# eflynn8/pharmacophore-diffusion

Measured on AMD Instinct MI355X. Metric: denoising steps/sec (batch x T) at 256-atom pocket, 6 centers, higher is better.
Workload: dtype f32; 1 GPU; BASELINE config 2: 256-atom pocket, 6 centers, T=500 schedule, batch=32 per GPU, dev.yml network; batch_per_gpu=32, n_prot=256, n_pharm=6, T=500, parallelism=graphs sharded over 1 GPU(s), no data-path collective

## Files before the change

pharmacophore-diffusion_amd/csrc/pf_device.h:

```cpp
#pragma once
#include <stdint.h>

#define PF_S 128
#define PF_V 16
#define PF_R 16
#define PF_MAXF 64
#define PF_MAXK 16
#define PF_MAX_GVPS 8

enum { ET_FF = 0, ET_PF = 1, ET_FP = 2, ET_PP = 3 };

#if defined(__HIP_DEVICE_COMPILE__)
#define PF_AS1 __attribute__((address_space(1)))
#else
#define PF_AS1
#endif
typedef const float PF_AS1* pf_gcf;

struct GvpW {
    pf_gcf a_wh;
    pf_gcf a_wu;
    pf_gcf a_main;
    pf_gcf a_main_c;
    pf_gcf a_gate_c;
// ... 105 lines not shown
    const float4* xn;
    const float* h;
    const float* v;
    float* msg_s;
    float* msg_v;
    const GvpW* w;
    const float* pre;
    int n_gvps;
    float rbf_mu[PF_R];
    float rbf_inv_sigma;
    float* sv_z; float* sv_g; float* sv_v; size_t sv_stride;
    int bf16;
    pf_gcf rg[4];
    const int* reg; int nreg, regB, ngroups4, ngroups8;
    pf_gcf rgs[4]; int rgs_stride;
    const float* zs;
    const float* ptab;
    int ptab_gstride;
    const int* ptype;
    const int* eorig;
    const int* l0_gid;
    const float* l0c;
    int ngroups_sel;
    const int* need; int need_stamp;
    int pa_abs;
    pf_gcf n16[4]; int n16_stride[4];
    int uni_base[3], uni_s01, uni_s2g, uni_pa_groups;
    int ptab16_off[4];
    const float* pcen; int pcen_nf;
    const float* x0_static;
    const int* pa_skip;
    int* cnt_snap;
    int* pa_gstamp; int pa_serial;
};

#define L0H_WR 0
#define L0H_WSH 2048
#define L0H_B 4224
#define L0H_WH0 4352
#define L0H_WU 4384
#define L0H_BG 4672
#define L0H_WHT 4736
#define L0H_WHT_PF 21120
#define L0H_B_PF 37504
#define L0H_SIZE (37504 + 128)
#define L0C_WHT_FF 0
#define L0C_B_FF 16384
#define L0C_WHT_FP 16512
#define L0C_B_FP 32896
#define L0C_SIZE (32896 + 128)
#define L0_NTAB 4
struct L0HoistParams {
    const float* src;
    float* l0c;
    const int* esrc; const int* edst; const float4* xn; int Epp;
    float rbf_mu0, rbf_mu_step, rbf_inv_sigma;
    float* zs;
    const float* enc_w; const float* enc_b; const float* enc_lw; const float* enc_lb;
    int rec_nf, nt;
    const float* t_dev;
    float t_host[64];
    float* ptab;
    const float* prot_h0; int Np; int* ptype; int* flag;
};

struct NodeW {
// ... 280 lines not shown
```

pharmacophore-diffusion_amd/csrc/pf_host.cpp:

```cpp
#include <hip/hip_runtime.h>

#include <algorithm>
#include <cmath>
#include <cstdio>
#include <cstdlib>
#include <cstring>
#include <ctime>
#include <map>
#include <string>
#include <unordered_map>
#include <climits>
#include <vector>

#include "../../include/pfdyn.h"
#include "pf_device.h"
#include "pf_bind.h"
#include "pf_pack.h"
#include "pf_train.h"
#include "pf_score.h"

using namespace pfpack;

#define L0_PTAB_SLOTS 2048

// ... 75 lines not shown
void pfk_drop_masks(const TrainCommon* c, uint32_t stream, int n_elems, float* out, hipStream_t s);
void pfk_pp_radius(const float4* xn, const int* prot_ptr, int B, float r2, int maxn, int* deg, const int* row_off,
                   int* src, int* dst, int pass, hipStream_t s);
void pfk_wide_encode(const WideEncParams* p, hipStream_t s);
void pfk_wide_pack(const float* flat, const WidePackJob* jobs, int n_jobs, float* out, hipStream_t s);
void pfk_wide_edge(const WideEdgeParams* p, int train, hipStream_t s);
void pfk_wide_node(const WideNodeParams* p, int train, hipStream_t s);
void pfk_wt_chain(const WtChainParams* p, int edge, int wgrad, hipStream_t s);
void pfk_wt_norm(const WtNormParams* p, int wgrad, hipStream_t s);
void pfk_wt_head_out(const WtHeadOutParams* p, int wgrad, hipStream_t s);
void pfk_wt_encode(const WtEncParams* p, int wgrad, hipStream_t s);
void pfk_wt_center_sum(const WtCenterSumParams* p, hipStream_t s);
void pfk_wt_reduce(const float* gpart, int gstride, float* grad, int nparams, hipStream_t s);
}

namespace {

static std::string g_create_error;

static void linspace_f32(float start, float end, int steps, float* out) {
    const float step = (end - start) / (float)(steps - 1);
    const int half = steps / 2;
    for (int i = 0; i < steps; ++i) out[i] = i < half ? start + step * (float)i : end - step * (float)(steps - i - 1);
}

}

struct LaunchPolicy {
    static constexpr int kCUs = 256, kSIMDs = 4 * kCUs;
    int n16_mask = 7;
    int tail_graphs_max = 256;
    int xcd_split = 1;
    int edge_rec = 1;
    int node_static = 1;
    int node_xcds = 2;
    int fused_uni = 1;
    int xchg_sleep = 1, hsb_avoid = 0;
    int hs_build = 1;
    int tail_form = 4;
    long n16_fuse_rows_max = 20000;
    long n16_rows_max = 24000;
    int rg_rows_max = 1 << 30;
    int rg2_rows_min = 12000;
    int rg2_rows_min_node = 12000;
    int rg2p_rows_min = 11000;
    int rg2_rows_min_hoist = 30000;
    int l0_rga = 0, l0_rgp = 0;
    int rg_split_max = 128;
    int rg_split_max_node = 256;
    int rg_split_max_head = 512;
    int coop_edge_max = 256, coop_node_max = 1024;
    int coop2_edge_max = 12000, coop2_dense_max = 1024;
    int rg_mode(int ntiles) const {
        const long rows = (long)ntiles * 32;
        if (rows > rg_rows_max) return 0;
        return rows >= rg2_rows_min ? 2 : 1;
    }
    void from_env() {
        auto geti = [](const char* v, int& x) { if (const char* e = getenv(v)) x = atoi(e); };
        geti("PFDYN_COOP_EDGE_MAX", coop_edge_max); geti("PFDYN_COOP_NODE_MAX", coop_node_max);
        if (const char* e = getenv("PFDYN_COOP2_EDGE_MAX")) coop2_edge_max = coop2_dense_max = atoi(e);
        if (const char* e = getenv("PFDYN_RG_SPLIT_MAX")) rg_split_max = rg_split_max_node = rg_split_max_head = atoi(e);
        geti("PFDYN_RG_SPLIT_MAX_NODE", rg_split_max_node); geti("PFDYN_RG_SPLIT_MAX_HEAD", rg_split_max_head);
        geti("PFDYN_RG_ROWS_MAX", rg_rows_max);
        if (const char* e = getenv("PFDYN_RG2_ROWS_MIN")) rg2_rows_min = rg2_rows_min_hoist = rg2p_rows_min = rg2_rows_min_node = atoi(e);
        geti("PFDYN_RG2P_ROWS_MIN", rg2p_rows_min); geti("PFDYN_RG2_ROWS_MIN_NODE", rg2_rows_min_node); geti("PFDYN_RG2_ROWS_MIN_HOIST", rg2_rows_min_hoist);
        geti("PFDYN_L0_RGP", l0_rgp); geti("PFDYN_L0_RGA", l0_rga);
        for (const char* v : {"PFDYN_RG2_ROWS_MIN", "PFDYN_RG2P_ROWS_MIN", "PFDYN_RG2_ROWS_MIN_HOIST", "PFDYN_RG_SPLIT_MAX", "PFDYN_L0_RGA",
                              "PFDYN_L0_RGP", "PFDYN_RG_ROWS_MAX"})
            if (getenv(v)) n16_mask = 0;
        geti("PFDYN_N16", n16_mask);
        geti("PFDYN_TAIL_GRAPHS_MAX", tail_graphs_max);
        geti("PFDYN_XCD_SPLIT", xcd_split);
        geti("PFDYN_EDGE_REC", edge_rec);
        geti("PFDYN_NODE_XCDS", node_xcds); geti("PFDYN_NODE_STATIC", node_static); geti("PFDYN_HS_BUILD", hs_build); geti("PFDYN_FUSED_UNI", fused_uni); geti("PFDYN_XCHG_SLEEP", xchg_sleep); geti("PFDYN_HSB_AVOID", hsb_avoid);
        if (const char* e = getenv("PFDYN_TAIL_FORM")) tail_form = (e[0] == 'n' || atoi(e) == 16) ? 16 : 4;
        if (const char* e = getenv("PFDYN_N16_ROWS_MAX")) n16_rows_max = n16_fuse_rows_max = atol(e);
        if (const char* e = getenv("PFDYN_N16_FUSE_ROWS_MAX")) n16_fuse_rows_max = atol(e);
    }
};

enum RunKind { RUN_NONE = 0, RUN_PLAIN, RUN_PINNED, RUN_GUIDED };

struct pf_handle {
    LaunchPolicy pol;
    pf_config cfg{};
    bool spec = true, wide = false;
    WideGvp* d_wgvp = nullptr;
    std::string err;
    std::map<std::string, RawTensor> raw;
    bool committed = false;

    float* d_w = nullptr;
    PackLayout pk;
    GvpW* d_gvp = nullptr;
    std::vector<GvpW> h_gvp;
    int msg_base(int layer, int et) const { return ((layer * 4 + et) * cfg.n_message_gvps); }
    int upd_base(int layer, int nt) const { return n_msg_tot + (layer * 2 + nt) * cfg.n_update_gvps; }
    int head_base() const { return n_msg_tot + n_upd_tot; }
    int n_msg_tot = 0, n_upd_tot = 0;
    bool use_pre = true;

    bool have_batch = false;
    int B = 0, Np = 0, Nf = 0, N = 0;
    int64_t Epp = 0, Ecap = 0;
    std::vector<int> h_prot_ptr, h_pharm_ptr;
    std::vector<int> h_reg;
// ... 37 lines not shown
    bool share_ok = false;
    int share_check = 1;
    int* d_reg_share = nullptr;
    int* d_pa_static = nullptr;
    int* d_rep_base = nullptr;
    int* d_need = nullptr;
    int need_stamp = 0, edges_stamp = 0;
    long share_rows = 0;
    std::vector<int> h_share_start, h_share_cnt;
    bool share_disable = false;
    bool train_rg_node = true;
    bool train_rg_edge = true;
    bool train_rg_head = true;
    float *t_hsv_z = nullptr, *t_hsv_g = nullptr, *t_hsv_v = nullptr;
    bool t_head_saved = false;
    unsigned int* d_xchg = nullptr;
    int* d_xstat = nullptr;
    int* xstat_host = nullptr;
    int xstat_ack = 0;
    int xchg_fault = 0, xchg_poll_max = 0;
    bool cen_hoist = true;
    float *d_cen_h = nullptr, *d_cen_p = nullptr, *d_snap[2] = {nullptr, nullptr};
    unsigned int* d_xchg2 = nullptr;
    int snap_cur = -1;
    std::vector<float> t_plan; size_t plan_pos = 0;
    bool cen_valid = false; float cen_t = 0.f; uint64_t cen_wver = 0;
    bool last_cen = false;
    bool pa_spec = true;
    bool spec_valid = false; float spec_t = 0.f; uint64_t spec_wver = 0;
    int step_id = 2;
    int *d_pa_stamp = nullptr, *d_pa_same = nullptr;
    bool e0_saved = false; EdgeParams e0{}; EncodeParams ep0{}; int e0_groups = 0;
    int last_spec = 0;
    int* d_pa_cnt = nullptr;
    int pa_spec_split = 0;
    bool pa_check = false;
    int pa_serial = 0, spec_serial = 0;
    int* d_pa_gstamp = nullptr;
    unsigned long long* d_pa_chk = nullptr;
    bool no_fixed_shapes = false;
    ScaleArgs pend_scale{}; bool has_pend_scale = false;
    bool vjp_full_kernels = false;
    bool no_fix_fuse = false;
    bool train_bf16 = false;
    bool train_node_save = true;
    std::vector<float*> t_nsv_z, t_nsv_g, t_nsv_v;
    std::vector<char> t_node_saved;
    std::vector<int> t_grp;
    RunKind run = RUN_NONE;
    void* d_pin = nullptr; size_t pin_capacity = 0;
    int* d_pin_flags = nullptr; float *d_pin_x = nullptr, *d_pin_h = nullptr;
    float pin_feat_norm = 1.f;
    void* d_seed = nullptr; size_t seed_capacity = 0;
    float *d_seed_x = nullptr, *d_seed_h = nullptr;
    float seed_alpha = 1.f, seed_sigma = 0.f, seed_feat_norm = 1.f;
    bool seed_armed = false;
    void* d_restr = nullptr; size_t restr_capacity = 0;
    void* restr_stage = nullptr; size_t restr_stage_capacity = 0; hipEvent_t restr_ev = nullptr;
    int n_restr = 0;
    float guide_scale = 0.f, guide_clip = 0.f;
    void* d_guide = nullptr; size_t guide_capacity = 0;
    float *d_g0 = nullptr, *d_gjx = nullptr, *d_ggrad = nullptr, *d_gshift = nullptr, *d_gzero = nullptr, *d_genergy = nullptr, *d_gD = nullptr;
    bool guide_have = false;
    float* guide_traj_energy = nullptr;
    int max_np = 0, max_nf = 0;
    bool edges_built = false;
// ... 401 lines not shown
        size_t total = 0;
        auto frag = [](int n_out, int K) { return (size_t)((n_out + 15) / 16) * ((K + 3) / 4) * 64; };
        for_each_gvp(c, [&](const GvpSpec& g) {
            const int H = std::max(g.vi, g.vo);
            const int* o = &h->po.gvp[6 * tab.size()];
            WideGvp w{};
            w.wh = h->d_flat + o[0]; w.wu = h->d_flat + o[1]; w.bm = h->d_flat + o[3]; w.bg = h->d_flat + o[5];
            w.vi = g.vi; w.vo = g.vo; w.si = g.si; w.so = g.so;
            jobs.push_back({o[2], g.so, g.si + H, (int)total});
            total += frag(g.so, g.si + H);
            jobs.push_back({o[4], g.vo, g.so, (int)total});
            total += frag(g.vo, g.so);
            tab.push_back(w);
        });
        if (total >= (size_t)1 << 31) PF_FAIL(h, PF_ERR_ARG, "pf_train_set_family: the model is too large for the width-generic packing");
        if (h->d_wpk) { (void)hipFree(h->d_wpk); h->d_wpk = nullptr; }
        PF_HIP(h, hipMalloc((void**)&h->d_wpk, std::max<size_t>(total, 1) * sizeof(float)));
        PF_HIP(h, upload(&h->d_wpk_jobs, jobs));
        h->n_wpk_jobs = (int)jobs.size();
        for (size_t i = 0; i < tab.size(); ++i) { tab[i].wm = h->d_wpk + jobs[2 * i].dst; tab[i].wg = h->d_wpk + jobs[2 * i + 1].dst; }
        PF_HIP(h, upload(&h->d_wgvp, tab));
        h->wpk_version = ~0ull;
    }
    if (h->wpk_version != h->w_version) {
        pfk_wide_pack(h->d_flat, h->d_wpk_jobs, h->n_wpk_jobs, h->d_wpk, s);
        h->wpk_version = h->w_version;
    }
    return PF_OK;
}

static int run_dynamics_wide(pf_handle* h, float* eps_h, float* eps_x, hipStream_t s, const float* t_scalar, bool train = false) {
    const pf_config& c = h->cfg;
    h->tail_done = false; h->last_tail = 0; h->last_hoist = 0;
    h->cen_valid = false; h->last_cen = false; h->spec_valid = false; h->last_spec = 0; h->e0_saved = false;
    if (!train && h->share_ok && h->share_check == 0) (void)share_now(h);
    if (!train && h->share_check == 2)
        PF_FAIL(h, PF_ERR_ARG, "pf_set_pocket_groups: the claim made for this batch is false -- a graph differs from its representative in "
                               "coordinates or features (compared on the device); bind the batch again without the claim");
    const int rc = ensure_wide_pack(h, s);
    if (rc) return rc;
    const int S = c.n_hidden_scalars, V = c.vector_size;
    WideEncParams ep{};
    ep.Np = h->Np; ep.Nf = h->Nf; ep.S = S; ep.rec_nf = c.rec_nf; ep.pharm_nf = c.pharm_nf;
    ep.prot_h0 = h->d_prot_h0; ep.pharm_h = h->d_pharm_h;
    ep.t = t_scalar ? nullptr : h->d_t; ep.t_scalar = t_scalar ? *t_scalar : 0.f; ep.gid = h->d_gid;
    for (int nt = 0; nt < 2; ++nt) {
        ep.w[nt] = h->d_w + h->pk.enc_w[nt]; ep.b[nt] = h->d_w + h->pk.enc_b[nt];
        ep.ln_w[nt] = h->d_w + h->pk.enc_lw[nt]; ep.ln_b[nt] = h->d_w + h->pk.enc_lb[nt];
    }
    float* const* st_h = train ? h->wt.st_h : h->d_h;
    float* const* st_v = train ? h->wt.st_v : h->d_v;
    ep.h_out = st_h[0];
    { ProfScope ps(h, pf_handle::K_ENCODE, s); pfk_wide_encode(&ep, s); }
    if (!h->edges_built) {
        const BuildParams bp = build_params(h, false);
        { ProfScope ps(h, pf_handle::K_BUILD, s); pfk_build_edges(&bp, s); }
        build_done(h, false);
    }
    h->last_family.assign(c.n_convs, 64);
    if (train) pfk_copy(reinterpret_cast<const float*>(h->d_xn), h->wt.xkeep, (size_t)h->N * 4, s);
    int cur = 0;
    for (int l = 0; l < c.n_convs; ++l) {
        const bool last = l == c.n_convs - 1;
        const LayerTiles lt = layer_tiles(h, l);
        WideEdgeParams e{};
        e.tiles = lt.etiles; e.ntiles = lt.n_etiles;
        e.dyn_cnt = h->d_dyn_cnt; e.esrc = h->d_esrc; e.edst = h->d_edst; e.xn = h->d_xn;
// ... 105 lines not shown
    } else {
        L0HoistParams lp = l0_params(h);
        lp.nt = h->B; lp.t_dev = h->d_t; lp.ptab = h->d_ptab_pg;
        pfk_l0_hoist(&lp, 1, s);
        dc.l0_ptab = h->d_ptab_pg; dc.l0_gstride = L0_NTAB * c.rec_nf * PF_S;
    }
}
static void edge_n16_form(DynCall& dc, int l) {
    pf_handle* h = dc.h; EdgeParams& e = dc.e; const pf_config& c = h->cfg; const bool shared = dc.shared;
    for (int et = 0; et < 4; ++et) {
        e.n16[et] = h->d_w + (l > 0 ? h->pk.n16_msg[(size_t)l * 4 + et] : h->pk.n16_l0[et]);
        e.n16_stride[et] = (int)(l > 0 ? h->pk.n16_msg_stride : h->pk.n16_l0_stride[et]);
        e.ptab16_off[et] = et == ET_PP ? c.rec_nf * PF_S : (et == ET_PF ? 2 * c.rec_nf * PF_S : -1);
    }
    if (l == 0) { e.zs = nullptr; dc.rgp = 4; h->last_hoist = 16; }
    if (l == 0 && dc.step != nullptr && h->run != RUN_NONE && !h->coords_custom) {
        e.x0_static = h->d_prot_x0;
        if (dc.spec_have && pa_ahead_ok(h, e, shared)) { e.pa_skip = h->d_pa_same; h->last_spec = 1; }
    }
    if (l == 0 && dc.cen_have && h->pk.n16_l0h[ET_FF] != 0) {
        for (int et : {(int)ET_FF, (int)ET_FP}) { e.n16[et] = h->d_w + h->pk.n16_l0h[et]; e.n16_stride[et] = (int)h->pk.n16_l0h_stride[et]; }
        e.pcen = h->d_cen_p; e.pcen_nf = h->Nf; h->last_cen = true;
    }
    e.ngroups_sel = region_groups(h, shared, 0, e.nreg, 16);
    int stride[3], cap[3], grp[3] = {0, 0, 0};
    bool uni = l == 0 && h->pol.fused_uni && !shared && e.reg == h->d_reg && e.nreg == 4 * h->B && h->B <= 64 && !e.pa_abs && !e.need &&
               uniform_regions(h, 3, stride, cap);
    for (int et = 0; et < 3 && uni; ++et) { grp[et] = (cap[et] + 15) / 16; uni = grp[et] > 0 && grp[et] < 8; }
    if (uni) {
        for (int et = 0; et < 3; ++et) e.uni_base[et] = h->h_reg[(size_t)et * h->B];
        e.uni_s01 = stride[0] | (stride[1] << 16);
        e.uni_s2g = stride[2] | (grp[0] << 16) | (grp[1] << 19) | (grp[2] << 22) | ((h->B - 1) << 25);
        e.uni_pa_groups = region_groups(h, shared, 3 * h->B, 4 * h->B, 16);
    }
    dc.rg = 4;
    if (l == 0 && e.x0_static && pa_ahead_ok(h, e, shared)) {
        e.cnt_snap = h->d_pa_cnt;
        h->e0 = e; h->ep0 = dc.ep; h->e0_saved = true;
        h->e0_groups = region_groups(h, shared, 3 * h->B, 4 * h->B, 16);
    }
}
static void edge_launch(DynCall& dc, int l) {
    pf_handle* h = dc.h; hipStream_t s = dc.s; const pf_config& c = h->cfg; const bool train = dc.train;
    const bool last = dc.last = (l == c.n_convs - 1), pruned = dc.pruned = (l == prune_layer(h));
    EdgeParams& e = dc.e; int &rg = dc.rg, &rgp = dc.rgp;
    e = edge_params_base(h, l, last, pruned);
    e.h = train ? h->t_H[l] : h->d_h[dc.cur]; e.v = train ? h->t_V[l] : h->d_v[dc.cur];
    e.msg_s = train ? h->t_msg_s[l] : h->d_msg_s; e.msg_v = train ? h->t_msg_v[l] : h->d_msg_v;
    if (dc.fuse_l0node && l == 1) { e.msg_s = h->d_msg_s2; e.msg_v = h->d_msg_v2; }
    e.pre = (l == 0 && dc.pre_ready) ? h->d_pre : nullptr;
    if (train) { e.sv_z = h->t_sv_z[l]; e.sv_g = h->t_sv_g[l]; e.sv_v = h->t_sv_v[l]; e.sv_stride = (size_t)std::max<int64_t>(h->Ecap, 1); }
    const bool shared = dc.shared = dc.share && pruned && l == 0;
    if ((last || pruned) && h->rg_compact && (last ? 2 : 4) * h->B <= 1024) {
        e.reg = shared ? h->d_reg_share : h->d_reg; e.regB = h->B; e.nreg = (last ? 2 : 4) * h->B; e.pa_abs = shared ? 1 : 0;
        if (shared) { e.need = h->d_need; e.need_stamp = h->edges_stamp; }
        e.ngroups4 = region_groups(h, shared, 0, e.nreg, 4); e.ngroups8 = region_groups(h, shared, 0, e.nreg, 8);
    }
    if (train && h->train_bf16) e.bf16 = 1;
    rg = train ? ((h->train_rg_edge && h->train_rg_node && !h->train_bf16) ? h->pol.rg_mode(e.ntiles) : 0)
               : h->pol.rg_mode(shared ? (int)((h->share_rows + 31) / 32) : e.ntiles);
    rgp = 0;
    if (dc.hoist && l == 0 && rg) {
        e.zs = h->d_zs; e.ptab = dc.l0_ptab; e.ptab_gstride = dc.l0_gstride; e.ptype = h->d_ptype; e.eorig = h->d_eorig; e.l0_gid = h->d_gid; e.l0c = h->d_l0c;
        rgp = rg;
        if (e.nreg > 0 && pruned) {
            rg = shared ? ((h->share_rows >= h->pol.rg2_rows_min || (long)e.ntiles * 32 >= h->pol.rg2_rows_min_hoist) ? 2 : 1)
// ... 162 lines not shown
    else if (train && h->train_rg_node && h->pol.rg_mode(n.ntiles) > 0) {
        n.grp = 32; n.grp_pa = 32;
        if (h->train_node_save) node_save_levels(h, l, n);
        ProfScope ps(h, pf_handle::K_NODE_COOP, s); pfk_rg_node(&n, nullptr, nullptr, l == 0, h->pol.rg_mode(n.ntiles), 0, s);
    }
    else if (n.ntiles <= h->pol.coop_node_max && !train) { ProfScope ps(h, pf_handle::K_NODE_COOP, s); pfk_node_update_coop(&n, l == 0, s); }
    else { ProfScope ps(h, pf_handle::K_NODE, s); pfk_node_update(&n, l == 0, s); }
}
static void head_launch(DynCall& dc) {
    pf_handle* h = dc.h; hipStream_t s = dc.s; const pf_config& c = h->cfg; const bool train = dc.train;
    HeadParams hp = head_params(h, dc.eps_h, dc.eps_x);
    hp.h = train ? h->t_H[c.n_convs] : h->d_h[dc.cur]; hp.v = train ? h->t_V[c.n_convs] : h->d_v[dc.cur];
    if (train) h->t_head_saved = false;
    if (!dc.head_done && train && h->train_rg_head && !h->pk.rg_msg.empty() && h->Nf > 0) {
        UnitParams up{};
        up.s_in = hp.h + (size_t)h->Np * PF_S; up.v_in = hp.v + (size_t)h->Np * 48; up.s_out = dc.eps_h; up.v_out = dc.eps_x;
        up.n = h->Nf; up.kind = 3; up.n_gvps = c.n_noise_gvps; up.pharm_nf = c.pharm_nf;
        up.stream = h->d_w + h->pk.rg_upd[(size_t)(c.n_convs - 1) * 2 + 1]; up.skip_gvps = c.n_update_gvps;
        up.sv_z = h->t_hsv_z; up.sv_g = h->t_hsv_g; up.sv_v = h->t_hsv_v; up.sv_stride = (size_t)h->Nf;
        { ProfScope ps(h, pf_handle::K_HEAD, s); pfk_rg_unit(&up, s); }
        h->t_head_saved = true; dc.head_done = true;
    }
    if (!dc.head_done) { ProfScope ps(h, pf_handle::K_HEAD, s); if (hp.ntiles <= h->pol.coop_node_max) pfk_noise_head_coop(&hp, s); else pfk_noise_head(&hp, s); }
}
static int run_dynamics(pf_handle* h, float* eps_h, float* eps_x, hipStream_t s, const float* t_scalar = nullptr, bool train = false, const StepParams* step = nullptr) {
    if (train ? h->train_wide : h->wide) return run_dynamics_wide(h, eps_h, eps_x, s, t_scalar, train);
    const pf_config& c = h->cfg;
    h->tail_done = false; h->last_tail = 0;
    DynCall dc{};
    dc.h = h; dc.s = s; dc.eps_h = eps_h; dc.eps_x = eps_x; dc.t_scalar = t_scalar; dc.train = train; dc.step = step;
    dc.cen_have = !train && h->cen_valid && h->edges_built && t_scalar != nullptr && *t_scalar == h->cen_t && h->cen_wver == h->w_version;
    h->cen_valid = false; h->last_cen = false;
    dc.spec_have = !train && h->spec_valid && h->edges_built && t_scalar != nullptr && *t_scalar == h->spec_t && h->spec_wver == h->w_version;
    h->spec_valid = false; h->last_spec = 0; h->e0_saved = false;
    if (!train) n16_refresh(h, s);
    dc.ep = encode_params(h, t_scalar, train ? h->t_H[0] : h->d_h[0]);
    if (const int rc = dyn_prologue(dc)) return rc;
    dyn_hoist_prepare(dc);
    h->last_hoist = 0;
    dc.fuse_l0node = !train && dc.n16_batch && (long)h->n_edge_tiles_act * 32 <= h->pol.n16_fuse_rows_max && (h->pol.n16_mask & 4) && (h->pol.n16_mask & 1) && dc.hoist && c.n_convs == 2 && prune_layer(h) == 0 && c.pf_k > 0 &&
                     c.n_update_gvps >= 1 && h->rg_compact && 2 * h->B <= 1024 && h->d_msg_s2 != nullptr && h->pk.n16_fused[0] != 0;
    for (int l = 0; l < c.n_convs; ++l, dc.cur ^= 1) { edge_launch(dc, l); node_launch(dc, l); }
    head_launch(dc);
    h->edges_built = h->tail_done;
    hipError_t e = hipGetLastError();
    if (e != hipSuccess) PF_FAIL(h, PF_ERR_HIP, "kernel launch failed: %s", hipGetErrorString(e));
    return PF_OK;
}

struct ZeroBatch {
    ZeroList z{};
    hipStream_t s;
    explicit ZeroBatch(hipStream_t st) : s(st) {}
    void add(void* p, size_t nbytes) {
        if (!p || nbytes == 0) return;
        if (z.cnt == 8) flush();
        z.p[z.cnt] = p; z.nbytes[z.cnt] = nbytes; ++z.cnt;
    }
    void flush() { pfk_zero_multi(&z, s); z.cnt = 0; }
};

static int check_ready(pf_handle* h, bool need_batch) {
    if (!h) return PF_ERR_ARG;
    if (!h->committed) PF_FAIL(h, PF_ERR_STATE, "weights not committed (pf_commit_weights)");
    if (need_batch && !h->have_batch) PF_FAIL(h, PF_ERR_STATE, "no pocket batch set (pf_set_pocket_batch)");
    return PF_OK;
}
// ... 1930 lines not shown
    out[0] = out[1] = out[2] = out[3] = 0;
    PF_HIP(h, hipStreamSynchronize((hipStream_t)stream));
    const int B = h->B;
    if (h->spec_valid && h->d_pa_same && h->d_dyn_cnt) {
        std::vector<int> cnt((size_t)5 * B), same(B);
        PF_HIP(h, hipMemcpy(cnt.data(), h->d_dyn_cnt, (size_t)5 * B * 4, hipMemcpyDeviceToHost));
        PF_HIP(h, hipMemcpy(same.data(), h->d_pa_same, (size_t)B * 4, hipMemcpyDeviceToHost));
        for (int g = 0; g < B; ++g) {
            const int64_t c = cnt[(size_t)3 * B + g];
            out[1] += c;
            out[0] += std::min<int64_t>(c, (int64_t)std::min(same[g], 1 << 26) * 16);
        }
    }
    if (h->cen_valid) { out[2] = 1; out[3] = h->Nf; }
    return PF_OK;
}

int pf_debug_pa_check(pf_handle* h, int64_t* out, pf_stream stream) {
    int rc = check_ready(h, true);
    if (rc) return rc;
    if (!out) PF_FAIL(h, PF_ERR_ARG, "pf_debug_pa_check: null argument");
    out[0] = out[1] = out[2] = 0;
    PF_HIP(h, hipStreamSynchronize((hipStream_t)stream));
    if (h->d_pa_chk) {
        unsigned long long v[3];
        PF_HIP(h, hipMemcpy(v, h->d_pa_chk, sizeof(v), hipMemcpyDeviceToHost));
        for (int k = 0; k < 3; ++k) out[k] = (int64_t)v[k];
    }
    return PF_OK;
}

int pf_debug_kernel_family(pf_handle* h, int32_t layer, int32_t* rows_per_wave) {
    if (!h || !rows_per_wave) return PF_ERR_ARG;
    if (layer == (int)h->last_family.size() + 2 && layer > 2) {
        *rows_per_wave = h->last_spec;
        return PF_OK;
    }
    if (layer == (int)h->last_family.size() + 1 && layer > 1) {
        *rows_per_wave = h->last_cen ? 1 : 0;
        return PF_OK;
    }
    if (layer == (int)h->last_family.size() && layer > 0) {
        *rows_per_wave = h->last_tail;
        return PF_OK;
    }
    if (layer < 0 || layer >= (int)h->last_family.size()) PF_FAIL(h, PF_ERR_STATE, "pf_debug_kernel_family: no dynamics call yet, or bad layer");
    *rows_per_wave = h->last_family[layer];
    return PF_OK;
}

int pf_debug_last_eps(pf_handle* h, float* dev_eps_h, float* dev_eps_x, pf_stream stream) {
    int rc = check_ready(h, true);
    if (rc) return rc;
    hipStream_t s = (hipStream_t)stream;
    if (dev_eps_h) PF_HIP(h, hipMemcpyAsync(dev_eps_h, h->d_eps_h, (size_t)h->Nf * h->cfg.pharm_nf * 4, hipMemcpyDeviceToDevice, s));
    if (dev_eps_x) PF_HIP(h, hipMemcpyAsync(dev_eps_x, h->d_eps_x, (size_t)h->Nf * 3 * 4, hipMemcpyDeviceToDevice, s));
    return PF_OK;
}

int pf_debug_xchg_timeouts(pf_handle* h, int32_t* n) {
    if (!h || !n) return PF_ERR_ARG;
    *n = 0;
    if (!h->d_xstat) return PF_OK;
    PF_HIP(h, hipDeviceSynchronize());
    PF_HIP(h, hipMemcpy(n, h->d_xstat, sizeof(int32_t), hipMemcpyDeviceToHost));
    return PF_OK;
// ... 145 lines not shown
```

pharmacophore-diffusion_amd/csrc/pf_n16.hip:

```cpp
#include <hip/hip_runtime.h>
#include <type_traits>
#include <algorithm>
#include "pf_device.h"
#ifdef N16_STAMPS
#define N16_STAMP_GLOBALS 1
namespace {
__device__ unsigned long long* g_n16_stamps = nullptr;
__device__ int g_n16_stamp_off = 0;
__device__ int g_n16_stamp_kid = -1;
}
#define SB_STAMP(k)                                                                                                    \
    do {                                                                                                               \
        const int rb_ = (int)blockIdx.x - g_n16_stamp_off;                                                             \
        if ((k) < 16 && (threadIdx.x & 63) == 0 && g_n16_stamps && rb_ >= 0 && rb_ < 64 && (g_n16_stamp_kid < 0 || g_n16_stamp_kid == 3)) \
            g_n16_stamps[((size_t)rb_ * 4 + (threadIdx.x >> 6)) * 64 + 40 + (k)] = __builtin_amdgcn_s_memtime();       \
    } while (0)
#endif
#include "pf_stepbuild.h"

#include "pf_n16_core.h"

using namespace pfn16;

namespace {
// ... 65 lines not shown
        const int base = (item & 1) * 16;
        nv = __builtin_amdgcn_readfirstlane(min(16, nvalid - base));
        if (nv <= 0) return;
        et = __builtin_amdgcn_readfirstlane(t.et);
        e0 = t.e0 + base;
    }
#ifdef N16_TRACE
    if (g_n16_trace && threadIdx.x == 0) {
        g_n16_trace[(size_t)blockIdx.x * 4 + 0] = __builtin_amdgcn_s_memtime();
        g_n16_trace[(size_t)blockIdx.x * 4 + 2] = (unsigned long long)__builtin_amdgcn_s_getreg((31 << 11) | (0 << 6) | 4);
        g_n16_trace[(size_t)blockIdx.x * 4 + 3] = (unsigned long long)__builtin_amdgcn_s_getreg((31 << 11) | (0 << 6) | 20) | ((unsigned long long)et << 32) | ((unsigned long long)nv << 40);
    }
#endif
    N16_CUT_AT(EDGE_CUT, 1, (float)(e0 + nv), p.msg_s);
    if constexpr (L0) {
        if (et == ET_PP && p.need) {
            const int e = e0 + min(lane & 15, nv - 1);
            if (!__any(p.need[p.edst[e]] == p.need_stamp)) return;
        }
        const int e = e0 + min(lane & 15, nv - 1);
        const int src = p.esrc[e], dst = p.edst[e];
        if (et == ET_PP || et == ET_PF || p.pcen) n16_edge_item<N16_M0H>(p, ep, &lds, e, src, dst, nv, et, lane, wq, sk);
        else n16_edge_item<N16_M0Z>(p, ep, &lds, e, src, dst, nv, et, lane, wq, sk);
    } else {
        const int e = e0 + min(lane & 15, nv - 1);
        n16_edge_item<N16_M0F>(p, ep, &lds, e, p.esrc[e], p.edst[e], nv, et, lane, wq, sk);
    }
#ifdef N16_TRACE
    if (g_n16_trace && threadIdx.x == 0) g_n16_trace[(size_t)blockIdx.x * 4 + 1] = __builtin_amdgcn_s_memtime();
#endif
}

__global__ __launch_bounds__(256) void k_n16_edge_u(const int* __restrict__ a_dyn_cnt, const int* __restrict__ a_esrc,
                                                    const int* __restrict__ a_edst, const int a_b0, const int a_b1, const int a_b2,
                                                    const int a_s01, const int a_s2g, const int* __restrict__ a_reg,
                                                    const EdgeParams p, const EncodeParams ep) {
    __shared__ N16Lds lds;
    const int lane = threadIdx.x & 63;
    const int wq = __builtin_amdgcn_readfirstlane((int)(threadIdx.x >> 6));
    const int j = lane & 15;
    int sk = 0;
    N16_STAMP(sk, lane, wq);
#ifdef N16_STAMPS
    struct WgTimes { __device__ ~WgTimes() { if (on) g_n16_stamps[(size_t)blockIdx.x * 2 + 1] = __builtin_amdgcn_s_memrealtime(); } bool on; } wgt_;
    wgt_.on = g_n16_stamp_kid == 100 && g_n16_stamps && threadIdx.x == 0 && blockIdx.x < 8192;
    if (wgt_.on) g_n16_stamps[(size_t)blockIdx.x * 2] = __builtin_amdgcn_s_memrealtime();
#endif
    const int gff = (a_s2g >> 16) & 7, gpf = (a_s2g >> 19) & 7, gfp = (a_s2g >> 22) & 7, a_B = (int)((unsigned)a_s2g >> 25) + 1;
    const int nff = a_B * gff, npf = a_B * gpf, nfp = a_B * gfp;
    int w = (int)blockIdx.x;
    if (p.cnt_snap && w == 0 && threadIdx.x < 64 && lane < a_B) p.cnt_snap[lane] = a_dyn_cnt[3 * a_B + lane];
#ifdef EDGE_U_SWAP
    if (w < nff) w += nff + npf; else if (w >= nff + npf && w < nff + npf + nfp) w -= nff + npf;
#endif
    if (w < nff + npf + nfp) {
        int et, base, stride, gk;
        if (w < nff) { et = ET_FF; base = a_b0; stride = a_s01 & 0xffff; gk = gff; }
        else if (w < nff + npf) { w -= nff; et = ET_PF; base = a_b1; stride = (int)((unsigned)a_s01 >> 16); gk = gpf; }
        else { w -= nff + npf; et = ET_FP; base = a_b2; stride = a_s2g & 0xffff; gk = gfp; }
        const int g = w / gk, k = w - g * gk;
        const int e0 = base + g * stride + 16 * k;
        const int cnt = a_dyn_cnt[et * a_B + g];
        const int src_raw = a_esrc[e0 + j], dst_raw = a_edst[e0 + j];
        const int nv = __builtin_amdgcn_readfirstlane(min(16, cnt - 16 * k));
        if (nv <= 0) return;
        const int jj = min(j, nv - 1);
        const int from = 4 * ((lane & 48) | jj);
        const int src = __builtin_amdgcn_ds_bpermute(from, src_raw), dst = __builtin_amdgcn_ds_bpermute(from, dst_raw);
        if (et == ET_PF || p.pcen) n16_edge_item<N16_M0H>(p, ep, &lds, e0 + jj, src, dst, nv, et, lane, wq, sk);
        else n16_edge_item<N16_M0Z>(p, ep, &lds, e0 + jj, src, dst, nv, et, lane, wq, sk);
        return;
    }
    w -= nff + npf + nfp;
    const int r = 3 * a_B + min(lane, a_B - 1);
    const int c = lane < a_B ? a_dyn_cnt[r] : 0;
    const int keep = p.pa_skip ? min(p.pa_skip[min(lane, a_B - 1)], (c + 15) >> 4) : 0;
    const int rs = a_reg[r];
    const int ng = ((c + 15) >> 4) - keep;
    int incl = ng;
    incl += dpp_i<0x111>(incl); incl += dpp_i<0x112>(incl); incl += dpp_i<0x114>(incl); incl += dpp_i<0x118>(incl);
    incl += dpp_ir<0x142, 0xa>(incl); incl += dpp_ir<0x143, 0xc>(incl);
    const unsigned long long m = __ballot(incl > w);
    if (!m) return;
    const int l = __builtin_amdgcn_readfirstlane(__ffsll((long long)m) - 1);
    const int first = __builtin_amdgcn_readlane(incl - ng, l);
    const int cnt = __builtin_amdgcn_readlane(c, l), start = __builtin_amdgcn_readlane(rs, l);
    const int loc = (w - first + __builtin_amdgcn_readlane(keep, l)) << 4;
    const int e0 = start + loc;
    const int nv = __builtin_amdgcn_readfirstlane(min(16, cnt - loc));
    const int e = e0 + min(j, nv - 1);
    n16_edge_item<N16_M0H>(p, ep, &lds, e, a_esrc[e], a_edst[e], nv, (int)ET_PP, lane, wq, sk);
}

struct N16LnPre { float a, b; };
__device__ __forceinline__ N16LnPre n16_ln_request(pf_gcf w1, pf_gcf b1, pf_gcf w2, pf_gcf b2, const int lane, const int wq) {
    const int t = wq * 64 + lane;
    N16LnPre q;
    q.a = (t < 128 ? w1 : b1)[t & 127];
    q.b = (t < 128 ? w2 : b2)[t & 127];
    return q;
}
__device__ __forceinline__ void n16_ln_stage(const N16LnPre& q, N16Lds* lds, const int lane, const int wq) {
    const int t = wq * 64 + lane;
    lds->ln[t] = q.a;
    lds->ln[256 + t] = q.b;
}
template <bool FROM_LDS = false>
__device__ __forceinline__ void n16_layernorm(pf_gcf lw, pf_gcf lb, float (&XS)[32], float (&VB)[4], N16Lds* lds, const int lane, const int wq,
                                              const int which = 0) {
    const int g = lane >> 4;
    float sum = 0.f;
#pragma unroll
    for (int k = 0; k < 32; ++k) sum += XS[k];
    const float mean = gsum(sum) * (1.0f / 128.0f);
    float var = 0.f;
#pragma unroll
    for (int k = 0; k < 32; ++k) { const float c = XS[k] - mean; var = fmaf(c, c, var); }
    const float rstd = rsqf_(gsum(var) * (1.0f / 128.0f) + 1e-5f);
#pragma unroll
    for (int T = 0; T < 8; ++T) {
        f32x4 w, b;
        if constexpr (FROM_LDS) {
            w = *reinterpret_cast<const f32x4*>(&lds->ln[256 * which + 16 * T + 4 * g]);
            b = *reinterpret_cast<const f32x4*>(&lds->ln[256 * which + 128 + 16 * T + 4 * g]);
// ... 551 lines not shown
    for (int c = 0; c < 3; ++c) in.xh[c] = msg ? p.v_in[(size_t)row * vw + c] : 0.f;
    N16P XP;
    if (msg) {
        constexpr int OFF1 = n16_sched(N16_M0F).nq % N16_D;
        n16_split_rows(XS, XP);
        n16_block<N16_M0F, 0, false, true, false, false>(ring, XS, XP, VB, in, S, &lds, lane, wq, sk);
        for (int gi = 1; gi + 1 < p.n_gvps; ++gi) n16_block<N16_GEN, OFF1, false, true, true, false>(ring, XS, XP, VB, in, S, &lds, lane, wq, sk);
        n16_block<N16_GEN, OFF1, true, true, true>(ring, XS, XP, VB, in, S, &lds, lane, wq, sk);
    } else {
        n16_gen_run<0, false>(p.n_gvps - 1, ring, XS, XP, VB, in, S, &lds, lane, wq, sk);
        if (p.n_gvps > 1) n16_block<N16_GEN, 0, true, true, true>(ring, XS, XP, VB, in, S, &lds, lane, wq, sk);
        else { n16_split_rows(XS, XP); n16_block<N16_GEN, 0, true, true, false>(ring, XS, XP, VB, in, S, &lds, lane, wq, sk); }
    }
    N16_STAMP(sk, lane, wq);
    if (j < nv) {
        float* so = p.s_out + (size_t)row * 128 + 32 * wq + 4 * g;
        *reinterpret_cast<f32x4*>(so) = S[0];
        *reinterpret_cast<f32x4*>(so + 16) = S[1];
        if (wq < 3) {
#pragma unroll
            for (int r = 0; r < 4; ++r) p.v_out[(size_t)row * 48 + (4 * g + r) * 3 + wq] = VB[r];
        }
    }
}

}

extern "C" {
void pfk_n16_edge(const EdgeParams* p, const EncodeParams* enc, int layer0, hipStream_t s) {
    if (p->ntiles == 0) return;
    const int grid = p->nreg > 0 ? p->ngroups_sel : p->ntiles * 2;
    if (grid <= 0) return;
    const EncodeParams noenc{};
    if (layer0 && p->uni_s2g != 0) {
        const int B = p->regB;
        const int nstat = B * (((p->uni_s2g >> 16) & 7) + ((p->uni_s2g >> 19) & 7) + ((p->uni_s2g >> 22) & 7));
        hipLaunchKernelGGL(k_n16_edge_u, dim3(nstat + p->uni_pa_groups), dim3(256), 0, s, p->dyn_cnt, p->esrc, p->edst, p->uni_base[0],
                           p->uni_base[1], p->uni_base[2], p->uni_s01, p->uni_s2g, p->reg, *p, *enc);
        return;
    }
    if (layer0) hipLaunchKernelGGL((k_n16_edge<true>), dim3(grid), dim3(256), 0, s, p->dyn_cnt, p->reg, p->nreg, p->regB, p->pa_abs, *p, *enc);
    else hipLaunchKernelGGL((k_n16_edge<false>), dim3(grid), dim3(256), 0, s, p->dyn_cnt, p->reg, p->nreg, p->regB, p->pa_abs, *p, noenc);
}
#ifdef N16_STAMPS
int pfk_n16_set_stamp_buffer(unsigned long long* dev, int off) {
    (void)hipMemcpyToSymbol(HIP_SYMBOL(g_n16_stamp_off), &off, sizeof(off));
    return (int)hipMemcpyToSymbol(HIP_SYMBOL(g_n16_stamps), &dev, sizeof(dev));
}
int pfk_n16_set_stamp_kernel(int kid) { return (int)hipMemcpyToSymbol(HIP_SYMBOL(g_n16_stamp_kid), &kid, sizeof(kid)); }
#endif
#ifdef N16_TRACE
int pfk_n16_set_trace_buffer(unsigned long long* dev) { return (int)hipMemcpyToSymbol(HIP_SYMBOL(g_n16_trace), &dev, sizeof(dev)); }
#endif
void pfk_n16_fused(const EdgeParams* p, const FusedParams* f, const EncodeParams* enc, hipStream_t s) {
    if (f->uni_groups != 0) {
        const int nffg = f->uni_groups & 255, npfg = (f->uni_groups >> 8) & 255;
        const int grid_u = 8 * std::max((f->B * nffg + f->B + 3) / 4, (f->B * npfg + 3) / 4);
        if (grid_u > 0)
            hipLaunchKernelGGL(k_n16_fused_u, dim3(grid_u), dim3(256), 0, s, p->dyn_cnt, p->esrc, p->edst, f->uni_ff_base, f->uni_pf_base,
                               f->uni_strides, f->uni_groups | (f->B << 16), *p, *f, *enc);
        return;
    }
    int grid = f->n_edge_items + f->B * (PF_MAXF / 16);
    if (f->xcd_split) grid = 8 * std::max((f->nff_cap + f->B + 3) / 4, (f->npf_cap + 3) / 4);
    if (grid <= 0) return;
    hipLaunchKernelGGL(k_n16_fused, dim3(grid), dim3(256), 0, s, p->dyn_cnt, p->reg, p->nreg, p->regB, *p, *f, *enc);
}
void pfk_n16_tail(const TailParams* t, const StepParams* sp, const BuildParams* bp, hipStream_t s) {
    if (sp->B <= 0) return;
    hipLaunchKernelGGL(k_n16_tail, dim3(sp->B), dim3(256), 0, s, bp->prot_ptr, bp->pharm_ptr, bp->reg, bp->B, bp->Np_tot, *t, *sp, *bp);
}
// ... 6 lines not shown
```

pharmacophore-diffusion_amd/csrc/pf_n16_core.h:

```cpp
#pragma once
#include <hip/hip_runtime.h>
#include <type_traits>
#include <algorithm>
#include "pf_device.h"

typedef float f32x4 __attribute__((ext_vector_type(4)));

namespace pfn16 {

template <int I, int N, class F>
__device__ __forceinline__ void static_for(F&& f) {
    if constexpr (I < N) {
        f(std::integral_constant<int, I>{});
        static_for<I + 1, N>(f);
    }
}

__device__ __forceinline__ float rcpf_(float x) { return __builtin_amdgcn_rcpf(x); }
__device__ __forceinline__ float sqrtf_(float x) { return __builtin_amdgcn_sqrtf(x); }
__device__ __forceinline__ float rsqf_(float x) { return __builtin_amdgcn_rsqf(x); }
__device__ __forceinline__ float sigmoidf_(float x) { return rcpf_(1.0f + __expf(-x)); }
__device__ __forceinline__ float siluf_(float x) { return x * rcpf_(1.0f + __expf(-x)); }

__device__ __forceinline__ f32x4 mfma16(const float a, const float b, const f32x4 c) {
// ... 448 lines not shown
        for (int r = 0; r < 4; ++r) {
            const float ze = (d - fmaf((float)(4 * g + r), mu_step, p.rbf_mu[0])) * p.rbf_inv_sigma;
            in.rb[r] = __expf(-(ze * ze));
        }
    }
    N16_STAMP(sk, lane, wq);
    N16P XP;
    if constexpr (KIND0 != N16_M0H) n16_split_rows(XS, XP);
    n16_block<KIND0, 0, false, true, false, false>(ring, XS, XP, VB, in, S, lds, lane, wq, sk);
    for (int gi = 1; gi + 1 < p.n_gvps; ++gi) n16_block<N16_GEN, OFF1, false, true, true, false>(ring, XS, XP, VB, in, S, lds, lane, wq, sk);
    n16_block<N16_GEN, OFF1, true, true, true>(ring, XS, XP, VB, in, S, lds, lane, wq, sk);
    N16_STAMP(sk, lane, wq);
    const SegMask16 sm = seg_masks16(rw.dst, j);
    const int dnext = dpp_i<0x101>(rw.dst);
    const bool tail = (j == nv - 1) | ((j < nv - 1) & (dnext != rw.dst));
#pragma unroll
    for (int t = 0; t < 2; ++t)
#pragma unroll
        for (int r = 0; r < 4; ++r) S[t][r] = seg_scan16(S[t][r], sm);
#pragma unroll
    for (int r = 0; r < 4; ++r) VB[r] = seg_scan16(VB[r], sm);
    if (tail) {
        float* ms = p.msg_s + (size_t)rw.e * PF_S + 32 * wq + 4 * g;
        *reinterpret_cast<f32x4*>(ms) = S[0];
        *reinterpret_cast<f32x4*>(ms + 16) = S[1];
        if (wq < 3) {
            float* mv = p.msg_v + (size_t)rw.e * 48 + 12 * g + wq;
#pragma unroll
            for (int r = 0; r < 4; ++r) mv[3 * r] = VB[r];
        }
    }
}

template <int KIND0>
__device__ __forceinline__ void n16_edge_item(const EdgeParams& p, const EncodeParams& ep, N16Lds* lds, const int e, const int src,
                                              const int dst, const int nv, const int et, const int lane, const int wq, int& sk) {
    N16_STAMP(sk, lane, wq);
    N16Ring ring;
    ring_start(ring, p.n16[et] + (size_t)wq * p.n16_stride[et], lane);
    const int g = lane >> 4;
    N16Rows rw;
    rw.e = e;
    rw.dst = dst;
    if (et == ET_PP && p.x0_static) {
        const float* a = p.x0_static + (size_t)src * 3;
        const float* b = p.x0_static + (size_t)rw.dst * 3;
        rw.xs = make_float4(a[0], a[1], a[2], 0.f); rw.xd = make_float4(b[0], b[1], b[2], 0.f);
    } else { rw.xs = p.xn[src]; rw.xd = p.xn[rw.dst]; }
    float XS[32], VB[4];
    f32x4 S[2];
    S[0] = (f32x4){0.f, 0.f, 0.f, 0.f}; S[1] = S[0];
    if constexpr (KIND0 == N16_M0H) {
        pf_gcf tp;
        if (et == ET_PP || et == ET_PF) {
            int ty = p.ptype[src] * PF_S + p.ptab16_off[et];
            if (p.ptab_gstride) ty += p.l0_gid[src] * p.ptab_gstride;
            tp = (pf_gcf)p.ptab + ty;
        } else tp = (pf_gcf)p.pcen + ((size_t)(et == ET_FP ? p.pcen_nf : 0) + (size_t)(src - ep.Np)) * PF_S;
        tp += 32 * wq + 4 * g;
        S[0] = *reinterpret_cast<const f32x4 PF_AS1*>(tp);
        S[1] = *reinterpret_cast<const f32x4 PF_AS1*>(tp + 16);
    }
    if constexpr (KIND0 == N16_M0Z) {
        const float tt = ep.t ? ((pf_gcf)ep.t)[((const int PF_AS1*)ep.gid)[src]] : ep.t_scalar;
        n16_encode_pharm(ep, (pf_gcf)ep.pharm_h + (size_t)(src - ep.Np) * ep.pharm_nf, tt, XS, lds, lane, wq);
    }
    if constexpr (KIND0 == N16_M0F) {
        const f32x4 PF_AS1* hp = reinterpret_cast<const f32x4 PF_AS1*>((pf_gcf)p.h + (size_t)src * PF_S) + g;
#pragma unroll
        for (int T = 0; T < 8; ++T) {
            const f32x4 x = hp[4 * T];
#pragma unroll
            for (int r = 0; r < 4; ++r) XS[4 * T + r] = x[r];
        }
        pf_gcf vp = (pf_gcf)p.v + (size_t)src * 48 + 12 * g + (wq < 3 ? wq : 0);
#pragma unroll
        for (int r = 0; r < 4; ++r) { const float x = vp[3 * r]; VB[r] = wq < 3 ? x : 0.f; }
    } else {
#pragma unroll
        for (int r = 0; r < 4; ++r) VB[r] = 0.f;
    }
    N16_CUT_AT(EDGE_CUT, 2, XS[0] + VB[0] + S[0][0] + rw.xs.x + rw.xd.x, p.msg_s);
    n16_edge_chain<KIND0>(p, ring, rw, XS, VB, S, lds, nv, lane, wq, sk);
}

}
```

Baseline: 685,600 sample-steps/s.

## Front-load layer-0 edge table rows and endpoint data via lane shuffles

```diff
diff --git a/pharmacophore-diffusion_amd/csrc/pf_device.h b/pharmacophore-diffusion_amd/csrc/pf_device.h
--- a/pharmacophore-diffusion_amd/csrc/pf_device.h
+++ b/pharmacophore-diffusion_amd/csrc/pf_device.h
@@ -161,6 +161,8 @@
     const int* pa_skip;
     int* cnt_snap;
     int* pa_gstamp; int pa_serial;
+    int l0_front, l0_nf, l0_ntypes;
+    const int4* l0_rec;
 };
 
 #define L0H_WR 0
diff --git a/pharmacophore-diffusion_amd/csrc/pf_host.cpp b/pharmacophore-diffusion_amd/csrc/pf_host.cpp
--- a/pharmacophore-diffusion_amd/csrc/pf_host.cpp
+++ b/pharmacophore-diffusion_amd/csrc/pf_host.cpp
@@ -131,6 +131,7 @@
     int tail_graphs_max = 256;
     int xcd_split = 1;
     int edge_rec = 1;
+    int l0_front = 1;
     int node_static = 1;
     int node_xcds = 2;
     int fused_uni = 1;
@@ -171,7 +172,7 @@
         geti("PFDYN_N16", n16_mask);
         geti("PFDYN_TAIL_GRAPHS_MAX", tail_graphs_max);
         geti("PFDYN_XCD_SPLIT", xcd_split);
-        geti("PFDYN_EDGE_REC", edge_rec);
+        geti("PFDYN_EDGE_REC", edge_rec); geti("PFDYN_L0_FRONT", l0_front);
         geti("PFDYN_NODE_XCDS", node_xcds); geti("PFDYN_NODE_STATIC", node_static); geti("PFDYN_HS_BUILD", hs_build); geti("PFDYN_FUSED_UNI", fused_uni); geti("PFDYN_XCHG_SLEEP", xchg_sleep); geti("PFDYN_HSB_AVOID", hsb_avoid);
         if (const char* e = getenv("PFDYN_TAIL_FORM")) tail_form = (e[0] == 'n' || atoi(e) == 16) ? 16 : 4;
         if (const char* e = getenv("PFDYN_N16_ROWS_MAX")) n16_rows_max = n16_fuse_rows_max = atol(e);
@@ -275,6 +276,7 @@
     int *d_pa_stamp = nullptr, *d_pa_same = nullptr;
     bool e0_saved = false; EdgeParams e0{}; EncodeParams ep0{}; int e0_groups = 0;
     int last_spec = 0;
+    int last_front = 0;
     int* d_pa_cnt = nullptr;
     int pa_spec_split = 0;
     bool pa_check = false;
@@ -742,7 +744,7 @@
 static int run_dynamics_wide(pf_handle* h, float* eps_h, float* eps_x, hipStream_t s, const float* t_scalar, bool train = false) {
     const pf_config& c = h->cfg;
     h->tail_done = false; h->last_tail = 0; h->last_hoist = 0;
-    h->cen_valid = false; h->last_cen = false; h->spec_valid = false; h->last_spec = 0; h->e0_saved = false;
+    h->cen_valid = false; h->last_cen = false; h->spec_valid = false; h->last_spec = 0; h->last_front = 0; h->e0_saved = false;
     if (!train && h->share_ok && h->share_check == 0) (void)share_now(h);
     if (!train && h->share_check == 2)
         PF_FAIL(h, PF_ERR_ARG, "pf_set_pocket_groups: the claim made for this batch is false -- a graph differs from its representative in "
@@ -914,6 +916,14 @@
         e.uni_s01 = stride[0] | (stride[1] << 16);
         e.uni_s2g = stride[2] | (grp[0] << 16) | (grp[1] << 19) | (grp[2] << 22) | ((h->B - 1) << 25);
         e.uni_pa_groups = region_groups(h, shared, 3 * h->B, 4 * h->B, 16);
+        const int nf = h->h_pharm_ptr[1] - h->h_pharm_ptr[0];
+        bool front = h->pol.l0_front != 0 && c.rec_nf <= 16 && nf >= 1 && nf <= 16;
+        for (int g = 0; g < h->B && front; ++g) front = h->h_pharm_ptr[g] == g * nf && h->h_pharm_ptr[g + 1] == (g + 1) * nf;
+        if (front) {
+            e.l0_front = e.pcen ? 3 : 1; e.l0_nf = nf; e.l0_ntypes = c.rec_nf;
+            e.l0_rec = h->rec_valid ? h->d_rec : nullptr;
+            h->last_front = e.l0_front | (e.l0_rec ? 4 : 0);
+        }
     }
     dc.rg = 4;
     if (l == 0 && e.x0_static && pa_ahead_ok(h, e, shared)) {
@@ -1142,7 +1152,7 @@
     dc.cen_have = !train && h->cen_valid && h->edges_built && t_scalar != nullptr && *t_scalar == h->cen_t && h->cen_wver == h->w_version;
     h->cen_valid = false; h->last_cen = false;
     dc.spec_have = !train && h->spec_valid && h->edges_built && t_scalar != nullptr && *t_scalar == h->spec_t && h->spec_wver == h->w_version;
-    h->spec_valid = false; h->last_spec = 0; h->e0_saved = false;
+    h->spec_valid = false; h->last_spec = 0; h->last_front = 0; h->e0_saved = false;
     if (!train) n16_refresh(h, s);
     dc.ep = encode_params(h, t_scalar, train ? h->t_H[0] : h->d_h[0]);
     if (const int rc = dyn_prologue(dc)) return rc;
@@ -3139,6 +3149,10 @@
 
 int pf_debug_kernel_family(pf_handle* h, int32_t layer, int32_t* rows_per_wave) {
     if (!h || !rows_per_wave) return PF_ERR_ARG;
+    if (layer == (int)h->last_family.size() + 3 && layer > 3) {
+        *rows_per_wave = h->last_front;
+        return PF_OK;
+    }
     if (layer == (int)h->last_family.size() + 2 && layer > 2) {
         *rows_per_wave = h->last_spec;
         return PF_OK;
diff --git a/pharmacophore-diffusion_amd/csrc/pf_n16.hip b/pharmacophore-diffusion_amd/csrc/pf_n16.hip
--- a/pharmacophore-diffusion_amd/csrc/pf_n16.hip
+++ b/pharmacophore-diffusion_amd/csrc/pf_n16.hip
@@ -121,13 +121,16 @@
 }
 
 __global__ __launch_bounds__(256) void k_n16_edge_u(const int* __restrict__ a_dyn_cnt, const int* __restrict__ a_esrc,
-                                                    const int* __restrict__ a_edst, const int a_b0, const int a_b1, const int a_b2,
-                                                    const int a_s01, const int a_s2g, const int* __restrict__ a_reg,
+                                                    const int4* __restrict__ a_rec, const long long a_b01, const int a_b2,
+                                                    const int a_s01, const int a_s2g, const int a_fe, const int* __restrict__ a_reg,
                                                     const EdgeParams p, const EncodeParams ep) {
     __shared__ N16Lds lds;
     const int lane = threadIdx.x & 63;
     const int wq = __builtin_amdgcn_readfirstlane((int)(threadIdx.x >> 6));
     const int j = lane & 15;
+    const int* a_edst = a_esrc + (a_fe & 0x3fffffff);
+    const int a_b0 = (int)(unsigned)a_b01, a_b1 = (int)(unsigned)((unsigned long long)a_b01 >> 32);
+    const bool front = (a_fe & (1 << 30)) != 0, front_cen = a_fe < 0;
     int sk = 0;
     N16_STAMP(sk, lane, wq);
 #ifdef N16_STAMPS
@@ -150,6 +153,47 @@
         const int g = w / gk, k = w - g * gk;
         const int e0 = base + g * stride + 16 * k;
         const int cnt = a_dyn_cnt[et * a_B + g];
+        if (front && (et == ET_PF || front_cen)) {
+            const bool rec = a_rec != nullptr && et != ET_FP;
+            int4 r0 = make_int4(0, 0, 0, 0), r1 = r0;
+            int src_raw = 0, dst_raw = 0;
+            if (rec) { const int4* rp = a_rec + (size_t)3 * (e0 + j); r0 = rp[0]; r1 = rp[1]; }
+            else { src_raw = a_esrc[e0 + j]; dst_raw = a_edst[e0 + j]; }
+            N16Pre pre;
+            ring_start(pre.ring, p.n16[et] + (size_t)wq * p.n16_stride[et], lane);
+            const int c0 = g * p.l0_nf, jc = min(j, p.l0_nf - 1);
+            if (et == ET_PF)
+                n16_rowq_request(pre.tq, (pf_gcf)p.ptab + (p.ptab_gstride ? (size_t)g * p.ptab_gstride : 0) + p.ptab16_off[ET_PF],
+                                 min(j, p.l0_ntypes - 1), lane, wq);
+            else n16_rowq_request(pre.tq, (pf_gcf)p.pcen + (size_t)(et == ET_FP ? p.pcen_nf : 0) * PF_S, c0 + jc, lane, wq);
+            float4 cx = make_float4(0.f, 0.f, 0.f, 0.f);
+            if (!rec) cx = p.xn[ep.Np + c0 + jc];
+            const int nv = __builtin_amdgcn_readfirstlane(min(16, cnt - 16 * k));
+            if (nv <= 0) return;
+            const int jj = min(j, nv - 1);
+            const int from = 4 * ((lane & 48) | jj);
+            const int cen0 = ep.Np + c0;
+            int src, dst;
+            if (rec) {
+                r0.x = __builtin_amdgcn_ds_bpermute(from, r0.x); r0.y = __builtin_amdgcn_ds_bpermute(from, r0.y);
+                r0.z = __builtin_amdgcn_ds_bpermute(from, r0.z); r0.w = __builtin_amdgcn_ds_bpermute(from, r0.w);
+                r1.x = __builtin_amdgcn_ds_bpermute(from, r1.x); r1.y = __builtin_amdgcn_ds_bpermute(from, r1.y);
+                r1.z = __builtin_amdgcn_ds_bpermute(from, r1.z); r1.w = __builtin_amdgcn_ds_bpermute(from, r1.w);
+                pre.xs = make_float4(__builtin_bit_cast(float, r0.x), __builtin_bit_cast(float, r0.y), __builtin_bit_cast(float, r0.z), 0.f);
+                pre.xd = make_float4(__builtin_bit_cast(float, r1.x), __builtin_bit_cast(float, r1.y), __builtin_bit_cast(float, r1.z), 0.f);
+                src = r0.w & 0xffffff; dst = r1.w;
+                pre.srow = et == ET_PF ? (int)((unsigned)r0.w >> 24) : src - cen0;
+            } else {
+                src = __builtin_amdgcn_ds_bpermute(from, src_raw); dst = __builtin_amdgcn_ds_bpermute(from, dst_raw);
+                const int fs = 4 * ((lane & 48) | ((src - cen0) & 15)), fd = 4 * ((lane & 48) | ((dst - cen0) & 15));
+                if (et == ET_PF) { pre.xs = p.xn[src]; pre.srow = p.ptype[src]; }
+                else { pre.xs = make_float4(n16_pickf(cx.x, fs), n16_pickf(cx.y, fs), n16_pickf(cx.z, fs), 0.f); pre.srow = src - cen0; }
+                if (et == ET_FP) pre.xd = p.xn[dst];
+                else pre.xd = make_float4(n16_pickf(cx.x, fd), n16_pickf(cx.y, fd), n16_pickf(cx.z, fd), 0.f);
+            }
+            n16_edge_item<N16_M0H>(p, ep, &lds, e0 + jj, src, dst, nv, et, lane, wq, sk, false, nullptr, &pre);
+            return;
+        }
         const int src_raw = a_esrc[e0 + j], dst_raw = a_edst[e0 + j];
         const int nv = __builtin_amdgcn_readfirstlane(min(16, cnt - 16 * k));
         if (nv <= 0) return;
@@ -178,7 +222,13 @@
     const int e0 = start + loc;
     const int nv = __builtin_amdgcn_readfirstlane(min(16, cnt - loc));
     const int e = e0 + min(j, nv - 1);
-    n16_edge_item<N16_M0H>(p, ep, &lds, e, a_esrc[e], a_edst[e], nv, (int)ET_PP, lane, wq, sk);
+    const int src = a_esrc[e], dst = a_edst[e];
+    N16RowQ tq;
+    tq.t[0] = (f32x4){0.f, 0.f, 0.f, 0.f}; tq.t[1] = tq.t[0];
+    if (front)
+        n16_rowq_request(tq, (pf_gcf)p.ptab + (p.ptab_gstride ? (size_t)l * p.ptab_gstride : 0) + p.ptab16_off[ET_PP], min(j, p.l0_ntypes - 1),
+                         lane, wq);
+    n16_edge_item<N16_M0H>(p, ep, &lds, e, src, dst, nv, (int)ET_PP, lane, wq, sk, front, &tq);
 }
 
 struct N16LnPre { float a, b; };
@@ -796,11 +846,14 @@
     const int grid = p->nreg > 0 ? p->ngroups_sel : p->ntiles * 2;
     if (grid <= 0) return;
     const EncodeParams noenc{};
-    if (layer0 && p->uni_s2g != 0) {
+    const long long ed = p->edst - p->esrc;
+    if (layer0 && p->uni_s2g != 0 && ed >= 0 && ed < (1ll << 30)) {
         const int B = p->regB;
         const int nstat = B * (((p->uni_s2g >> 16) & 7) + ((p->uni_s2g >> 19) & 7) + ((p->uni_s2g >> 22) & 7));
-        hipLaunchKernelGGL(k_n16_edge_u, dim3(nstat + p->uni_pa_groups), dim3(256), 0, s, p->dyn_cnt, p->esrc, p->edst, p->uni_base[0],
-                           p->uni_base[1], p->uni_base[2], p->uni_s01, p->uni_s2g, p->reg, *p, *enc);
+        const long long b01 = (long long)(((unsigned long long)(unsigned)p->uni_base[1] << 32) | (unsigned)p->uni_base[0]);
+        const int fe = (int)((unsigned)ed | ((unsigned)(p->l0_front & 3) << 30));
+        hipLaunchKernelGGL(k_n16_edge_u, dim3(nstat + p->uni_pa_groups), dim3(256), 0, s, p->dyn_cnt, p->esrc, p->l0_front ? p->l0_rec : nullptr,
+                           b01, p->uni_base[2], p->uni_s01, p->uni_s2g, fe, p->reg, *p, *enc);
         return;
     }
     if (layer0) hipLaunchKernelGGL((k_n16_edge<true>), dim3(grid), dim3(256), 0, s, p->dyn_cnt, p->reg, p->nreg, p->regB, p->pa_abs, *p, *enc);
diff --git a/pharmacophore-diffusion_amd/csrc/pf_n16_core.h b/pharmacophore-diffusion_amd/csrc/pf_n16_core.h
--- a/pharmacophore-diffusion_amd/csrc/pf_n16_core.h
+++ b/pharmacophore-diffusion_amd/csrc/pf_n16_core.h
@@ -504,17 +504,39 @@
     }
 }
 
+struct N16RowQ { f32x4 t[2]; };
+__device__ __forceinline__ void n16_rowq_request(N16RowQ& q, pf_gcf table, const int row, const int lane, const int wq) {
+    pf_gcf tp = table + (size_t)row * PF_S + 32 * wq + 4 * (lane >> 4);
+    q.t[0] = *reinterpret_cast<const f32x4 PF_AS1*>(tp);
+    q.t[1] = *reinterpret_cast<const f32x4 PF_AS1*>(tp + 16);
+}
+__device__ __forceinline__ float n16_pickf(const float v, const int from) {
+    return __builtin_bit_cast(float, __builtin_amdgcn_ds_bpermute(from, __builtin_bit_cast(int, v)));
+}
+__device__ __forceinline__ void n16_rowq_pick(const N16RowQ& q, const int row, f32x4 (&S)[2], const int lane) {
+    const int from = 4 * ((lane & 48) | (row & 15));
+#pragma unroll
+    for (int t = 0; t < 2; ++t)
+#pragma unroll
+        for (int r = 0; r < 4; ++r) S[t][r] = n16_pickf(q.t[t][r], from);
+}
+
+struct N16Pre { N16Ring ring; float4 xs, xd; N16RowQ tq; int srow; };
+
 template <int KIND0>
 __device__ __forceinline__ void n16_edge_item(const EdgeParams& p, const EncodeParams& ep, N16Lds* lds, const int e, const int src,
-                                              const int dst, const int nv, const int et, const int lane, const int wq, int& sk) {
+                                              const int dst, const int nv, const int et, const int lane, const int wq, int& sk,
+                                              const bool use_tab = false, const N16RowQ* tabq = nullptr, const N16Pre* pre = nullptr) {
     N16_STAMP(sk, lane, wq);
     N16Ring ring;
-    ring_start(ring, p.n16[et] + (size_t)wq * p.n16_stride[et], lane);
+    if (pre) ring = pre->ring;
+    else ring_start(ring, p.n16[et] + (size_t)wq * p.n16_stride[et], lane);
     const int g = lane >> 4;
     N16Rows rw;
     rw.e = e;
     rw.dst = dst;
-    if (et == ET_PP && p.x0_static) {
+    if (pre) { rw.xs = pre->xs; rw.xd = pre->xd; }
+    else if (et == ET_PP && p.x0_static) {
         const float* a = p.x0_static + (size_t)src * 3;
         const float* b = p.x0_static + (size_t)rw.dst * 3;
         rw.xs = make_float4(a[0], a[1], a[2], 0.f); rw.xd = make_float4(b[0], b[1], b[2], 0.f);
@@ -523,15 +545,19 @@
     f32x4 S[2];
     S[0] = (f32x4){0.f, 0.f, 0.f, 0.f}; S[1] = S[0];
     if constexpr (KIND0 == N16_M0H) {
-        pf_gcf tp;
-        if (et == ET_PP || et == ET_PF) {
-            int ty = p.ptype[src] * PF_S + p.ptab16_off[et];
-            if (p.ptab_gstride) ty += p.l0_gid[src] * p.ptab_gstride;
-            tp = (pf_gcf)p.ptab + ty;
-        } else tp = (pf_gcf)p.pcen + ((size_t)(et == ET_FP ? p.pcen_nf : 0) + (size_t)(src - ep.Np)) * PF_S;
-        tp += 32 * wq + 4 * g;
-        S[0] = *reinterpret_cast<const f32x4 PF_AS1*>(tp);
-        S[1] = *reinterpret_cast<const f32x4 PF_AS1*>(tp + 16);
+        if (pre) n16_rowq_pick(pre->tq, pre->srow, S, lane);
+        else if (use_tab) n16_rowq_pick(*tabq, p.ptype[src], S, lane);
+        else {
+            pf_gcf tp;
+            if (et == ET_PP || et == ET_PF) {
+                int ty = p.ptype[src] * PF_S + p.ptab16_off[et];
+                if (p.ptab_gstride) ty += p.l0_gid[src] * p.ptab_gstride;
+                tp = (pf_gcf)p.ptab + ty;
+            } else tp = (pf_gcf)p.pcen + ((size_t)(et == ET_FP ? p.pcen_nf : 0) + (size_t)(src - ep.Np)) * PF_S;
+            tp += 32 * wq + 4 * g;
+            S[0] = *reinterpret_cast<const f32x4 PF_AS1*>(tp);
+            S[1] = *reinterpret_cast<const f32x4 PF_AS1*>(tp + 16);
+        }
     }
     if constexpr (KIND0 == N16_M0Z) {
         const float tt = ep.t ? ((pf_gcf)ep.t)[((const int PF_AS1*)ep.gid)[src]] : ep.t_scalar;
```

Result: no change. 686,100 sample-steps/s, median of 4 (+0.1%).
